# AdrianoEttari/DiffusionRemoteSensing

Measured on AMD Instinct MI355X. Metric: unet_denoise_steps_per_s, higher is better.
Workload: dtype f16 main + block-scaled fp6 (e2m3) cross terms of tap pairs on the wide 3x3 layers (FL, 11 of 11 launches of the dominant kernel); split bf16 x3 (hi + lo) everywhere else; f32 accumulate

## Files before the change

diffusionremotesensing_amd/csrc/reverse_step.hip:

```cpp
#include "drs_common.h"
#include "step_update.h"

__global__ __launch_bounds__(256) void sampler_step_tab_kernel(float* __restrict__ x, const float* __restrict__ eps,
                                                               const float* __restrict__ noise, int t,
                                                               const float* __restrict__ alpha,
                                                               const float* __restrict__ alpha_hat,
                                                               const float* __restrict__ beta, int64_t numel) {
  const DrsAncestralCoef k = drs_ancestral_coef(alpha, alpha_hat, beta, t);
  for (int64_t i = (int64_t)blockIdx.x * blockDim.x + threadIdx.x; i < numel; i += (int64_t)gridDim.x * blockDim.x) {
    float v = drs_ancestral_update(k, x[i], eps[i]);
    if (noise) v = drs_ancestral_noise(k, v, noise[i]);
    x[i] = v;
  }
}

extern "C" int drs_sampler_step(float* x, const float* eps_pred, const float* noise, int t, const float* alpha,
                                const float* alpha_hat, const float* beta, int noise_steps, int64_t numel,
                                drs_stream_t stream) {
  DRS_REQUIRE(x && eps_pred && alpha && alpha_hat && beta, DRS_ERR_ARG, "sampler_step: null pointer");
  if (int st = drs_check_move("sampler_step", false, 0, t, 0, 0.f, noise_steps, noise, DRS_NOISE_OPTIONAL)) return st;
  if (numel <= 0) return DRS_OK;
  DRS_LAUNCH(sampler_step_tab_kernel, dim3(ew_blocks(numel)), dim3(256), 0, (hipStream_t)stream, x, eps_pred,
                     noise, t, alpha, alpha_hat, beta, numel);
  DRS_CHECK_HIP(hipGetLastError());
  return DRS_OK;
}

__global__ void sampler_step_cfg_kernel(float* __restrict__ x, const float* __restrict__ ec,
                                        const float* __restrict__ eu, float w, const float* __restrict__ noise, int t,
                                        const float* __restrict__ alpha, const float* __restrict__ alpha_hat,
                                        const float* __restrict__ beta, int64_t numel) {
  const DrsAncestralCoef k = drs_ancestral_coef(alpha, alpha_hat, beta, t);
  for (int64_t i = (int64_t)blockIdx.x * blockDim.x + threadIdx.x; i < numel; i += (int64_t)gridDim.x * blockDim.x) {
    float v = drs_ancestral_update(k, x[i], drs_cfg_lerp(eu[i], ec[i], w));
    if (noise) v = drs_ancestral_noise(k, v, noise[i]);
    x[i] = v;
  }
}
extern "C" int drs_sampler_step_cfg(float* x, const float* eps_cond, const float* eps_uncond, float cfg_scale,
                                    const float* noise, int t, const float* alpha, const float* alpha_hat,
                                    const float* beta, int noise_steps, int64_t numel, drs_stream_t stream) {
  DRS_REQUIRE(x && eps_cond && eps_uncond && alpha && alpha_hat && beta, DRS_ERR_ARG, "sampler_step_cfg: null pointer");
  if (int st = drs_check_move("sampler_step_cfg", false, 0, t, 0, 0.f, noise_steps, noise, DRS_NOISE_OPTIONAL)) return st;
  if (numel <= 0) return DRS_OK;
  DRS_LAUNCH(sampler_step_cfg_kernel, dim3(ew_blocks(numel)), dim3(256), 0, (hipStream_t)stream, x, eps_cond,
                     eps_uncond, cfg_scale, noise, t, alpha, alpha_hat, beta, numel);
  DRS_CHECK_HIP(hipGetLastError());
  return DRS_OK;
}

namespace {

__global__ __launch_bounds__(256) void ddim_step_kernel(float* __restrict__ x, const float* __restrict__ ec,
                                                        const float* __restrict__ eu, float w,
                                                        const float* __restrict__ noise, int t, int t_prev, float eta,
                                                        const float* __restrict__ alpha_hat, int64_t numel) {
  const DrsDdimCoef k = drs_ddim_coef(alpha_hat, t, t_prev, eta);
  const bool add_noise = noise != nullptr && k.has_sigma;
  for (int64_t i = (int64_t)blockIdx.x * blockDim.x + threadIdx.x; i < numel; i += (int64_t)gridDim.x * blockDim.x) {
    float e = ec[i];
    if (eu) e = drs_cfg_lerp(eu[i], e, w);
    float v = drs_ddim_update(k, x[i], e);
    if (add_noise) v = drs_ddim_noise(k, v, noise[i]);
    x[i] = v;
  }
}

__device__ __forceinline__ float cfg_lerp(float uncond, float cond, float w) {
#pragma clang fp contract(off)
  const float d = cond - uncond;
  return fabsf(w) < 0.5f ? fmaf(w, d, uncond) : fmaf(-(1.f - w), d, cond);
}

template <bool DDIM>
struct MoveCoef;
template <>
struct MoveCoef<false> {
  DrsAncestralCoef k;
  __device__ MoveCoef(const float* alpha, const float* alpha_hat, const float* beta, int t, int, float)
      : k(drs_ancestral_coef(alpha, alpha_hat, beta, t)) {}
  __device__ bool draws() const { return true; }
  __device__ float step(float x, float eps) const {
#pragma clang fp contract(off)
    return k.c_inv * fmaf(-k.c_eps, eps, x);
  }
  __device__ float add(float v, float z) const { return fmaf(k.c_sig, z, v); }
};
template <>
struct MoveCoef<true> {
  DrsDdimCoef k;
  __device__ MoveCoef(const float*, const float* alpha_hat, const float*, int t, int t_prev, float eta)
      : k(drs_ddim_coef(alpha_hat, t, t_prev, eta)) {}
  __device__ bool draws() const { return k.has_sigma; }
  __device__ float step(float x, float eps) const {
#pragma clang fp contract(off)
    const float p = k.a * x, q = k.b * eps;
    return p + q;
  }
  __device__ float add(float v, float z) const { return fmaf(k.s, z, v); }
};

struct InpaintArgs {
  float* x;
  const float* ec;
  const float* eu;
  float w;
  const float* noise;
  const float* known;
  const unsigned char* mask;
  int planes, C, Cm;
  int64_t hw;
  int t, t_prev;
  float eta;
  const float *alpha, *alpha_hat, *beta;
};

template <int V, bool DDIM>
__global__ __launch_bounds__(256) void inpaint_step_kernel(const InpaintArgs a) {
  const MoveCoef<DDIM> coef(a.alpha, a.alpha_hat, a.beta, a.t, a.t_prev, a.eta);
  const DrsKnownCoef kc(a.alpha_hat, a.t_prev);
  const bool add_noise = a.noise != nullptr && coef.draws();
  const bool to_zero = a.t_prev == 0;
  const int64_t groups = a.hw / V;
  for (int plane = blockIdx.y; plane < a.planes; plane += gridDim.y) {
    const int64_t base = (int64_t)plane * a.hw;
    const unsigned char* mp = a.mask + (a.Cm == 1 ? (int64_t)(plane / a.C) * a.hw : base);
    for (int64_t g = (int64_t)blockIdx.x * blockDim.x + threadIdx.x; g < groups; g += (int64_t)gridDim.x * blockDim.x) {
      const int64_t at = base + g * V;
      float xs[V], es[V], ks[V], zs[V];
      unsigned m;
      if constexpr (V == 4) {
        const float4 x4 = *reinterpret_cast<const float4*>(a.x + at);
        const float4 e4 = *reinterpret_cast<const float4*>(a.ec + at);
        const float4 k4 = *reinterpret_cast<const float4*>(a.known + at);
        xs[0] = x4.x; xs[1] = x4.y; xs[2] = x4.z; xs[3] = x4.w;
        es[0] = e4.x; es[1] = e4.y; es[2] = e4.z; es[3] = e4.w;
        ks[0] = k4.x; ks[1] = k4.y; ks[2] = k4.z; ks[3] = k4.w;
        if (a.eu) {
          const float4 u4 = *reinterpret_cast<const float4*>(a.eu + at);
          es[0] = cfg_lerp(u4.x, es[0], a.w); es[1] = cfg_lerp(u4.y, es[1], a.w);
          es[2] = cfg_lerp(u4.z, es[2], a.w); es[3] = cfg_lerp(u4.w, es[3], a.w);
        }
        if (a.noise) {
          const float4 z4 = *reinterpret_cast<const float4*>(a.noise + at);
          zs[0] = z4.x; zs[1] = z4.y; zs[2] = z4.z; zs[3] = z4.w;
        }
        m = *reinterpret_cast<const unsigned*>(mp + g * 4);
      } else {
        xs[0] = a.x[at];
        es[0] = a.ec[at];
        ks[0] = a.known[at];
        if (a.eu) es[0] = cfg_lerp(a.eu[at], es[0], a.w);
        if (a.noise) zs[0] = a.noise[at];
        m = mp[g];
      }
#pragma unroll
      for (int p = 0; p < V; ++p) {
        float v = coef.step(xs[p], es[p]);
        if (add_noise) v = coef.add(v, zs[p]);
        if ((m >> (8 * p)) & 0xffu) v = to_zero ? ks[p] : kc.at(ks[p], zs[p]);
        xs[p] = v;
      }
      if constexpr (V == 4) *reinterpret_cast<float4*>(a.x + at) = make_float4(xs[0], xs[1], xs[2], xs[3]);
      else a.x[at] = xs[0];
    }
  }
}

__device__ __forceinline__ float jump_to(float A, float x, float B, float z) {
#pragma clang fp contract(off)
  const float p = A * x, q = B * z;
  return p + q;
}

__global__ __launch_bounds__(256) void renoise_kernel(float* __restrict__ x, const float* __restrict__ z, int s, int t,
                                                      const float* __restrict__ alpha_hat, int64_t numel, bool vec) {
  const double r = (double)alpha_hat[t] / (double)alpha_hat[s];
  const float A = (float)sqrt(r), B = (float)sqrt(fmax(1.0 - r, 0.0));
  const int64_t tid = (int64_t)blockIdx.x * blockDim.x + threadIdx.x, stride = (int64_t)gridDim.x * blockDim.x;
  const int64_t groups = vec ? numel / 4 : 0;
  for (int64_t g = tid; g < groups; g += stride) {
    float4 v = reinterpret_cast<const float4*>(x)[g];
    const float4 n = reinterpret_cast<const float4*>(z)[g];
    v.x = jump_to(A, v.x, B, n.x);
    v.y = jump_to(A, v.y, B, n.y);
    v.z = jump_to(A, v.z, B, n.z);
    v.w = jump_to(A, v.w, B, n.w);
    reinterpret_cast<float4*>(x)[g] = v;
  }
  for (int64_t i = groups * 4 + tid; i < numel; i += stride) x[i] = jump_to(A, x[i], B, z[i]);
}

__global__ __launch_bounds__(256) void dpm_step_kernel(float* __restrict__ x, const float* __restrict__ ec,
                                                       const float* __restrict__ eu, float w, float* __restrict__ hist,
                                                       int t_q, int t, int t_p, const float* __restrict__ alpha_hat,
                                                       int64_t numel, bool vec) {
  const DrsDpmCoef k = drs_dpm_coef(alpha_hat, t_q, t, t_p);
  const int64_t tid = (int64_t)blockIdx.x * blockDim.x + threadIdx.x, stride = (int64_t)gridDim.x * blockDim.x;
  const int64_t groups = vec ? numel / 4 : 0;
  for (int64_t g = tid; g < groups; g += stride) {
    const float4 x4 = reinterpret_cast<const float4*>(x)[g];
    const float4 e4 = reinterpret_cast<const float4*>(ec)[g];
    float xs[4] = {x4.x, x4.y, x4.z, x4.w}, es[4] = {e4.x, e4.y, e4.z, e4.w}, hs[4] = {0.f, 0.f, 0.f, 0.f};
    if (eu) {
      const float4 u4 = reinterpret_cast<const float4*>(eu)[g];
      es[0] = drs_cfg_lerp(u4.x, es[0], w); es[1] = drs_cfg_lerp(u4.y, es[1], w);
      es[2] = drs_cfg_lerp(u4.z, es[2], w); es[3] = drs_cfg_lerp(u4.w, es[3], w);
    }
    if (k.second) {
      const float4 h4 = reinterpret_cast<const float4*>(hist)[g];
      hs[0] = h4.x; hs[1] = h4.y; hs[2] = h4.z; hs[3] = h4.w;
    }
#pragma unroll
    for (int p = 0; p < 4; ++p) {
      const float x0 = drs_dpm_x0(k, xs[p], es[p]);
      xs[p] = drs_dpm_update(k, xs[p], es[p], hs[p]);
      hs[p] = x0;
    }
    reinterpret_cast<float4*>(hist)[g] = make_float4(hs[0], hs[1], hs[2], hs[3]);
    reinterpret_cast<float4*>(x)[g] = make_float4(xs[0], xs[1], xs[2], xs[3]);
  }
  for (int64_t i = groups * 4 + tid; i < numel; i += stride) {
    float e = ec[i];
    if (eu) e = drs_cfg_lerp(eu[i], e, w);
    const float xv = x[i], h = k.second ? hist[i] : 0.f;
    hist[i] = drs_dpm_x0(k, xv, e);
    x[i] = drs_dpm_update(k, xv, e, h);
  }
}

template <bool DDIM>
int launch_inpaint(const InpaintArgs& a, hipStream_t s) {
  const bool wide = a.hw % 4 == 0 && aligned16(a.x) && aligned16(a.ec) && aligned16(a.known) && ((uintptr_t)a.mask & 3u) == 0 &&
                    (!a.eu || aligned16(a.eu)) && (!a.noise || aligned16(a.noise));
  const int gx = ew_blocks(wide ? a.hw / 4 : a.hw);
  int gy = 8192 / gx;
  if (gy > a.planes) gy = a.planes;
  if (gy < 1) gy = 1;
  if (wide) DRS_LAUNCH((inpaint_step_kernel<4, DDIM>), dim3(gx, gy), dim3(256), 0, s, a);
// ... 67 lines not shown
```

diffusionremotesensing_amd/csrc/small_kernels.hip:

```cpp
#include "drs_common.h"
#include <algorithm>

typedef unsigned u32x4 __attribute__((ext_vector_type(4)));

__global__ void pack_conv_kernel(const float* __restrict__ w, const float* __restrict__ b,
                                 const float* __restrict__ gamma, const float* __restrict__ beta,
                                 const float* __restrict__ rmean, const float* __restrict__ rvar, float eps,
                                 float* __restrict__ dst_w, float* __restrict__ dst_b, int Cout, int Cin, int taps,
                                 int transposed, int mfma_layout) {
  const int64_t total = (int64_t)Cout * Cin * taps;
  for (int64_t i = (int64_t)blockIdx.x * blockDim.x + threadIdx.x; i < total;
       i += (int64_t)gridDim.x * blockDim.x) {
    int tap, ci, co;
    if (mfma_layout) {
      ci = (int)(i % Cin);
      co = (int)((i / Cin) % Cout);
      tap = (int)(i / ((int64_t)Cin * Cout));
    } else {
      co = (int)(i % Cout);
      ci = (int)((i / Cout) % Cin);
      tap = (int)(i / ((int64_t)Cin * Cout));
    }
    const int64_t src = transposed ? (((int64_t)ci * Cout + co) * taps + tap) : (((int64_t)co * Cin + ci) * taps + tap);
    float v = w[src];
// ... 46 lines not shown
    const int c = (int)((i / hw) % C);
    const int n = (int)(i / (hw * C));
    dst[i] = src[((int64_t)n * hw + r) * src_cs + src_co + c];
  }
}
__global__ void sp_to_nchw_kernel(const char* __restrict__ src, float* __restrict__ dst, int N, int C, int H, int W,
                                  int src_cs, int src_co) {
  const int64_t total = (int64_t)N * C * H * W;
  const int64_t hw = (int64_t)H * W;
  const int gw = src_cs >= 32 ? 32 : src_cs;
  for (int64_t i = (int64_t)blockIdx.x * blockDim.x + threadIdx.x; i < total; i += (int64_t)gridDim.x * blockDim.x) {
    const int64_t r = i % hw;
    const int c = (int)((i / hw) % C) + src_co;
    const int n = (int)(i / (hw * C));
    const char* g = src + (((int64_t)n * hw + r) * src_cs + (c / gw) * gw) * 4;
    const __bf16 h = *reinterpret_cast<const __bf16*>(g + (c % gw) * 2);
    const __bf16 l = *reinterpret_cast<const __bf16*>(g + gw * 2 + (c % gw) * 2);
    dst[i] = (float)h + (float)l;
  }
}
__global__ void sp_add_rowvec_kernel(const char* __restrict__ src, char* __restrict__ dst, const float* __restrict__ vec,
                                     int vec_stride, int64_t slots, int64_t slots_per_image, int C) {
  typedef __bf16 bf16x8_t __attribute__((ext_vector_type(8)));
  const int spp = C / 8;
  for (int64_t i = (int64_t)blockIdx.x * blockDim.x + threadIdx.x; i < slots; i += (int64_t)gridDim.x * blockDim.x) {
    const int64_t pix = i / spp;
    const int sl = (int)(i % spp), grp = sl >> 2, kg = sl & 3;
    const int n = (int)(i / slots_per_image);
    const int64_t off = (pix * C + grp * 32) * 4 + kg * 16;
    const bf16x8_t h = *reinterpret_cast<const bf16x8_t*>(src + off), l = *reinterpret_cast<const bf16x8_t*>(src + off + 64);
    const float* v = vec + (int64_t)n * vec_stride + grp * 32 + kg * 8;
    float x[8];
#pragma unroll
    for (int j = 0; j < 8; ++j) x[j] = (float)h[j] + (float)l[j] + v[j];
    u32x4 oh, ol;
#pragma unroll
    for (int q = 0; q < 4; ++q) { const uint2 s_ = drs_split2(x[2 * q], x[2 * q + 1]); oh[q] = s_.x; ol[q] = s_.y; }
    *reinterpret_cast<u32x4*>(dst + off) = oh;
    *reinterpret_cast<u32x4*>(dst + off + 64) = ol;
  }
}
int drs_launch_nchw_to_nhwc(const float* src, float* dst, int N, int C, int H, int W, int dst_cs, int dst_co,
                            hipStream_t s) {
  DRS_LAUNCH(nchw_to_nhwc_kernel, dim3(ew_blocks((int64_t)N * C * H * W)), dim3(256), 0, s, src, dst, N, C, H,
                     W, dst_cs, dst_co);
  DRS_CHECK_HIP(hipGetLastError());
  return DRS_OK;
}
int drs_launch_sp_to_nchw(const float* src, float* dst, int N, int C, int H, int W, int src_cs, int src_co,
                          hipStream_t s) {
  DRS_LAUNCH(sp_to_nchw_kernel, dim3(ew_blocks((int64_t)N * C * H * W)), dim3(256), 0, s,
                     reinterpret_cast<const char*>(src), dst, N, C, H, W, src_cs, src_co);
  DRS_CHECK_HIP(hipGetLastError());
  return DRS_OK;
}
int drs_launch_sp_add_rowvec(const float* src, float* dst, const float* vec, int vec_stride, int N, long long pix_per_image,
                             int C, hipStream_t s) {
  DRS_REQUIRE(C % 32 == 0, DRS_ERR_SHAPE, "sp_add_rowvec: C=%d", C);
  const int64_t per_image = (int64_t)pix_per_image * (C / 8), slots = per_image * N;
  if (slots == 0) return DRS_OK;
  DRS_LAUNCH(sp_add_rowvec_kernel, dim3(ew_blocks(slots)), dim3(256), 0, s, reinterpret_cast<const char*>(src),
                     reinterpret_cast<char*>(dst), vec, vec_stride, slots, per_image, C);
  DRS_CHECK_HIP(hipGetLastError());
  return DRS_OK;
}
int drs_launch_nhwc_to_nchw(const float* src, float* dst, int N, int C, int H, int W, int src_cs, int src_co,
                            hipStream_t s) {
  DRS_LAUNCH(nhwc_to_nchw_kernel, dim3(ew_blocks((int64_t)N * C * H * W)), dim3(256), 0, s, src, dst, N, C, H,
                     W, src_cs, src_co);
  DRS_CHECK_HIP(hipGetLastError());
  return DRS_OK;
}

__global__ __launch_bounds__(256) void conv3x3_planar_kernel(const float* __restrict__ in, const float* __restrict__ w,
                                                             const float* __restrict__ b,
                                                             const float* __restrict__ res, float* __restrict__ out,
                                                             int N, int Cin, int Cout, int H, int W, int relu) {
  constexpr int kW = kMaxBands * kMaxBands * 9;
  __shared__ float sw[kW + kMaxBands];
  for (int i = threadIdx.x; i < Cout * Cin * 9; i += blockDim.x) sw[i] = w[i];
  if (threadIdx.x < Cout) sw[kW + threadIdx.x] = b ? b[threadIdx.x] : 0.f;
  __syncthreads();
  const int64_t hw = (int64_t)H * W;
  const int64_t total = (int64_t)N * hw;
  for (int64_t p = (int64_t)blockIdx.x * blockDim.x + threadIdx.x; p < total; p += (int64_t)gridDim.x * blockDim.x) {
    const int x = (int)(p % W);
    const int y = (int)((p / W) % H);
    const int n = (int)(p / hw);
#pragma unroll 1
    for (int c0 = 0; c0 < Cout; c0 += 4) {
      const int nc = min(4, Cout - c0);
      const float* swc = sw + c0 * Cin * 9;
      float acc[4];
#pragma unroll
      for (int co = 0; co < 4; ++co) acc[co] = co < nc ? sw[kW + c0 + co] : 0.f;
      for (int ci = 0; ci < Cin; ++ci) {
        const float* ip = in + ((int64_t)n * Cin + ci) * hw;
#pragma unroll
        for (int ky = 0; ky < 3; ++ky) {
          const int iy = y + ky - 1;
          if (iy < 0 || iy >= H) continue;
#pragma unroll
          for (int kx = 0; kx < 3; ++kx) {
            const int ix = x + kx - 1;
            if (ix < 0 || ix >= W) continue;
            const float a = ip[(int64_t)iy * W + ix];
#pragma unroll
            for (int co = 0; co < 4; ++co)
              if (co < nc) acc[co] = fmaf(a, swc[(co * Cin + ci) * 9 + ky * 3 + kx], acc[co]);
          }
        }
      }
#pragma unroll
      for (int co = 0; co < 4; ++co) {
        if (co >= nc) break;
        float v = acc[co];
        if (relu) v = drs_maxf(v, 0.f);
        const int64_t o = ((int64_t)n * Cout + c0 + co) * hw + (int64_t)y * W + x;
        if (res) v += res[o];
        out[o] = v;
      }
    }
  }
}
int drs_launch_conv3x3_planar(const float* in, const float* w, const float* b, const float* res, float* out, int N,
                              int Cin, int Cout, int H, int W, int relu, hipStream_t s) {
  DRS_REQUIRE(Cin >= 1 && Cin <= kMaxBands && Cout >= 1 && Cout <= kMaxBands, DRS_ERR_SHAPE,
              "planar conv: Cin=%d Cout=%d (max %d)", Cin, Cout, kMaxBands);
  DRS_LAUNCH(conv3x3_planar_kernel, dim3(ew_blocks((int64_t)N * H * W)), dim3(256), 0, s, in, w, b, res, out,
                     N, Cin, Cout, H, W, relu);
  DRS_CHECK_HIP(hipGetLastError());
  return DRS_OK;
}

constexpr int kStemRows = 4;
constexpr int kStemBpc = 2;
__device__ __attribute__((aligned(16))) float stem_zero_line[4];
template <int COUT>
__global__ __launch_bounds__(256, kStemBpc) void stem_kernel(const float* __restrict__ in, const float* __restrict__ w,
                                                             const float* __restrict__ b, const float* __restrict__ res,
                                                             int res_batch, float* __restrict__ out, int N, int Cin, int H,
                                                             int W, int out_sp) {
  static_assert(COUT == 16, "a pixel is 64 bytes in both output formats");
  constexpr int R = kStemRows;
  constexpr int kB = COUT * kMaxBands * 9;
  __shared__ __attribute__((aligned(16))) float sw[kB + COUT];
  __shared__ __attribute__((aligned(16))) char sT[4][64 * 64];
  for (int i = threadIdx.x; i < COUT * Cin * 9; i += blockDim.x) {
    const int co = i / (Cin * 9), r = i % (Cin * 9), ci = r / 9, tap = r % 9;
    sw[(tap * Cin + ci) * COUT + co] = w[i];
  }
  if (threadIdx.x < COUT) sw[kB + threadIdx.x] = b[threadIdx.x];
  __syncthreads();
  const int lane = threadIdx.x & 63, wave = threadIdx.x >> 6;
  char* tb = sT[wave];
  const int sw_px = (lane >> 2) & 3;
  const int lin_q = (lane & 3) ^ ((lane >> 4) & 3);
  const int lin_off = (lane >> 2) * 64 + lin_q * 16;
  const int64_t hw = (int64_t)H * W;
  const int xbs = (W + 63) / 64, ygs = (H + R - 1) / R;
  const int units = N * ygs * xbs;
  for (int u = blockIdx.x * 4 + wave; u < units; u += gridDim.x * 4) {
    const int xb = u % xbs, yg = (u / xbs) % ygs, n = u / (xbs * ygs);
    const int x0 = xb * 64, x = x0 + lane, y0 = yg * R;
    const int npx = min(64, W - x0);
    float acc[R][COUT];
#pragma unroll
    for (int o = 0; o < R; ++o)
#pragma unroll
      for (int co = 0; co < COUT; ++co) acc[o][co] = sw[kB + co];
    u32x4 rnext[4] = {};
    auto load_res = [&](int o) __attribute__((always_inline)) {
      const int y = min(y0 + o, H - 1);
      const char* rp = reinterpret_cast<const char*>(res + (res_batch == 1 ? ((int64_t)y * W + x0) : ((int64_t)n * H + y) * W + x0) * COUT);
#pragma unroll
      for (int j = 0; j < 4; ++j)
        rnext[j] = *reinterpret_cast<const u32x4*>((j * 16 + (lane >> 2) < npx) ? rp + j * 1024 + lin_off
                                                                                 : reinterpret_cast<const char*>(stem_zero_line));
    };
    if (res) load_res(0);
#pragma unroll 1
    for (int ci = 0; ci < Cin; ++ci) {
      const float* ip = in + ((int64_t)n * Cin + ci) * hw;
      float a[R + 2][3];
#pragma unroll
      for (int r = 0; r < R + 2; ++r) {
        const int iy = y0 - 1 + r;
        const bool yok = iy >= 0 && iy < H;
        const float* rowp = ip + (int64_t)iy * W;
#pragma unroll
        for (int kx = 0; kx < 3; ++kx) {
          const int ix = x - 1 + kx;
          a[r][kx] = *((yok && ix >= 0 && ix < W) ? rowp + ix : stem_zero_line);
        }
      }
#pragma unroll
      for (int ky = 0; ky < 3; ++ky)
#pragma unroll
        for (int kx = 0; kx < 3; ++kx) {
          const float* wr = &sw[((ky * 3 + kx) * Cin + ci) * COUT];
          float wv[COUT];
#pragma unroll
          for (int co = 0; co < COUT; co += 4) {
            const float4 q = *reinterpret_cast<const float4*>(wr + co);
            wv[co] = q.x; wv[co + 1] = q.y; wv[co + 2] = q.z; wv[co + 3] = q.w;
          }
#pragma unroll
          for (int o = 0; o < R; ++o)
#pragma unroll
            for (int co = 0; co < COUT; ++co) acc[o][co] = fmaf(a[o + ky][kx], wv[co], acc[o][co]);
        }
    }
#pragma unroll
    for (int o = 0; o < R; ++o) {
      const int y = y0 + o;
      if (y >= H) break;
      const int64_t p0 = ((int64_t)n * H + y) * W + x0;
      if (res) {
        const u32x4 rv[4] = {rnext[0], rnext[1], rnext[2], rnext[3]};
        if (o + 1 < R) load_res(o + 1);
#pragma unroll
        for (int j = 0; j < 4; ++j) *reinterpret_cast<u32x4*>(tb + j * 1024 + lane * 16) = rv[j];
        asm volatile("s_waitcnt lgkmcnt(0)" ::: "memory");
#pragma unroll
        for (int q = 0; q < 4; ++q) {
          const float4 r4 = *reinterpret_cast<const float4*>(tb + lane * 64 + ((q ^ sw_px) << 4));
          acc[o][q * 4] += r4.x; acc[o][q * 4 + 1] += r4.y; acc[o][q * 4 + 2] += r4.z; acc[o][q * 4 + 3] += r4.w;
        }
        asm volatile("s_waitcnt lgkmcnt(0)" ::: "memory");
      }
      if (out_sp) {
#pragma unroll
        for (int co = 0; co < COUT; co += 8) {
          u32x4 h, l;
#pragma unroll
          for (int q = 0; q < 4; ++q) { const uint2 s_ = drs_split2(acc[o][co + 2 * q], acc[o][co + 2 * q + 1]); h[q] = s_.x; l[q] = s_.y; }
          *reinterpret_cast<u32x4*>(tb + lane * 64 + (((co >> 3) ^ sw_px) << 4)) = h;
          *reinterpret_cast<u32x4*>(tb + lane * 64 + (((2 + (co >> 3)) ^ sw_px) << 4)) = l;
        }
      } else {
#pragma unroll
        for (int co = 0; co < COUT; co += 4)
          *reinterpret_cast<float4*>(tb + lane * 64 + (((co >> 2) ^ sw_px) << 4)) = make_float4(acc[o][co], acc[o][co + 1], acc[o][co + 2], acc[o][co + 3]);
      }
      asm volatile("s_waitcnt lgkmcnt(0)" ::: "memory");
      char* op = reinterpret_cast<char*>(out + p0 * COUT);
#pragma unroll
      for (int j = 0; j < 4; ++j) {
        const u32x4 v = *reinterpret_cast<const u32x4*>(tb + j * 1024 + lane * 16);
        if (j * 16 + (lane >> 2) < npx) *reinterpret_cast<u32x4*>(op + j * 1024 + lin_off) = v;
      }
      asm volatile("s_waitcnt lgkmcnt(0)" ::: "memory");
    }
  }
}
int drs_launch_stem(const float* in_nchw, const float* w, const float* b, const float* res_nhwc, int res_batch,
                    float* out_nhwc, int N, int Cin, int Cout, int H, int W, hipStream_t s, int out_sp) {
  DRS_REQUIRE(Cout == 16 && Cin >= 1 && Cin <= kMaxBands, DRS_ERR_SHAPE, "stem: Cin=%d Cout=%d unsupported (Cin max %d)", Cin,
              Cout, kMaxBands);
  const int64_t units = (int64_t)N * ((H + kStemRows - 1) / kStemRows) * ((W + 63) / 64);
  if (units == 0) return DRS_OK;
  DRS_REQUIRE(units < (1LL << 31), DRS_ERR_SHAPE, "stem: %lld row segments", (long long)units);
  const int64_t blocks = std::min<int64_t>((units + 3) / 4, 16384);
  DRS_LAUNCH(stem_kernel<16>, dim3((unsigned)blocks), dim3(256), 0, s, in_nchw, w, b, res_nhwc,
                     res_batch, out_nhwc, N, Cin, H, W, out_sp);
  DRS_CHECK_HIP(hipGetLastError());
  return DRS_OK;
}

__device__ __forceinline__ void cubic_coeffs(float t, float c[4]) {
  const float A = -0.75f;
  const float x0 = t + 1.f, x1 = t, x2 = 1.f - t, x3 = 2.f - t;
  c[0] = ((A * x0 - 5.f * A) * x0 + 8.f * A) * x0 - 4.f * A;
  c[1] = ((A + 2.f) * x1 - (A + 3.f)) * x1 * x1 + 1.f;
  c[2] = ((A + 2.f) * x2 - (A + 3.f)) * x2 * x2 + 1.f;
  c[3] = ((A * x3 - 5.f * A) * x3 + 8.f * A) * x3 - 4.f * A;
}
__global__ __launch_bounds__(256) void bicubic_kernel(const float* __restrict__ x, float* __restrict__ y, int NC, int H,
                                                      int W, int scale) {
  const int OH = H * scale, OW = W * scale;
  const int64_t total = (int64_t)NC * OH * OW;
  const float rs = 1.f / (float)scale;
  for (int64_t i = (int64_t)blockIdx.x * blockDim.x + threadIdx.x; i < total; i += (int64_t)gridDim.x * blockDim.x) {
    const int ox = (int)(i % OW);
    const int oy = (int)((i / OW) % OH);
    const int64_t nc = i / ((int64_t)OW * OH);
    const float sy = rs * ((float)oy + 0.5f) - 0.5f;
    const float sx = rs * ((float)ox + 0.5f) - 0.5f;
    const float fy = floorf(sy), fx = floorf(sx);
    const int iy = (int)fy, ix = (int)fx;
    float cy[4], cx[4];
    cubic_coeffs(sy - fy, cy);
    cubic_coeffs(sx - fx, cx);
    const float* ip = x + nc * (int64_t)H * W;
    float acc = 0.f;
#pragma unroll
    for (int a = 0; a < 4; ++a) {
      const int yy = min(max(iy - 1 + a, 0), H - 1);
      float row = 0.f;
#pragma unroll
      for (int bq = 0; bq < 4; ++bq) {
        const int xx = min(max(ix - 1 + bq, 0), W - 1);
        row = fmaf(ip[(int64_t)yy * W + xx], cx[bq], row);
      }
      acc = fmaf(row, cy[a], acc);
    }
    y[i] = acc;
  }
}
int drs_launch_bicubic(const float* x, float* y, int N, int C, int H, int W, int scale, hipStream_t s) {
  DRS_REQUIRE(scale >= 1, DRS_ERR_SHAPE, "bicubic: scale=%d", scale);
  DRS_LAUNCH(bicubic_kernel, dim3(ew_blocks((int64_t)N * C * H * W * scale * scale)), dim3(256), 0, s, x, y,
                     N * C, H, W, scale);
  DRS_CHECK_HIP(hipGetLastError());
  return DRS_OK;
}

__global__ __launch_bounds__(256) void time_mlp_kernel(const int64_t* __restrict__ t, const float* __restrict__ inv_freq,
                                                       const float* __restrict__ W1, const float* __restrict__ b1,
                                                       const float* __restrict__ W2, const float* __restrict__ b2,
                                                       float* __restrict__ out, int out_stride, int dim_in,
                                                       int dim_out) {
  extern __shared__ __attribute__((aligned(16))) float smem[];
  float* e = smem;
  float* h = smem + dim_in;
  const int b = blockIdx.x;
  const float tf = (float)t[b];
  const int half = dim_in / 2;
  for (int j = threadIdx.x; j < half; j += blockDim.x) {
    const float arg = tf * inv_freq[j];
    e[j] = sinf(arg);
    e[half + j] = cosf(arg);
  }
  __syncthreads();
  for (int c = threadIdx.x; c < dim_out; c += blockDim.x) {
    const float* wr = W1 + (int64_t)c * dim_in;
    float acc = 0.f;
    for (int k = 0; k < dim_in; ++k) acc = fmaf(wr[k], e[k], acc);
    acc += b1[c];
    h[c] = acc / (1.f + expf(-acc));
  }
  __syncthreads();
  for (int c = threadIdx.x; c < dim_out; c += blockDim.x) {
    const float* wr = W2 + (int64_t)c * dim_out;
    float acc = 0.f;
    for (int k = 0; k < dim_out; ++k) acc = fmaf(wr[k], h[k], acc);
    acc += b2[c];
    out[(int64_t)b * out_stride + c] = drs_maxf(acc, 0.f);
  }
}
int drs_launch_time_mlp(const int64_t* t, const float* inv_freq, const float* W1, const float* b1, const float* W2,
                        const float* b2, float* out, int out_stride, int B, int dim_in, int dim_out, hipStream_t s) {
  DRS_REQUIRE(dim_in % 2 == 0 && dim_in > 0 && dim_out > 0, DRS_ERR_SHAPE, "time_mlp: dims %d %d", dim_in, dim_out);
  if (B == 0) return DRS_OK;
  const size_t shmem = (size_t)(dim_in + dim_out) * sizeof(float);
  DRS_LAUNCH(time_mlp_kernel, dim3(B), dim3(256), shmem, s, t, inv_freq, W1, b1, W2, b2, out, out_stride,
                     dim_in, dim_out);
  DRS_CHECK_HIP(hipGetLastError());
  return DRS_OK;
}

__global__ __launch_bounds__(256) void time_mlp_multi_kernel(const int64_t* __restrict__ t,
                                                             const float* __restrict__ inv_freq,
                                                             const char* __restrict__ packed,
                                                             const long long* __restrict__ table,
                                                             float* __restrict__ out, int out_stride, int dim_in,
                                                             const float* __restrict__ label_emb,
                                                             const long long* __restrict__ labels, int label_batch,
                                                             int num_classes) {
  extern __shared__ __attribute__((aligned(16))) float smem[];
  float* e = smem;
  float* h = smem + dim_in;
  const int b = blockIdx.x;
// ... 200 lines not shown
```

diffusionremotesensing_amd/csrc/upfuse_proj_sp.hip:

```cpp
#include <stdio.h>
#include <stdlib.h>

#include "conv_epilogue.h"
#include "mfma_policy.h"

namespace {

constexpr int RBC = 8;
struct RowOpU { PolicyBF16X3::Frag c, e; };

__device__ __forceinline__ bf16x8 dpp_shift_u(const bf16x8& edge, const bf16x8& own, bool left) {
  const u32x4 e = __builtin_bit_cast(u32x4, edge), r = __builtin_bit_cast(u32x4, own);
  u32x4 o;
#pragma unroll
  for (int j = 0; j < 4; ++j)
    o[j] = left ? (unsigned)__builtin_amdgcn_update_dpp((int)e[j], (int)r[j], 0x111, 0xf, 0xf, false)
                : (unsigned)__builtin_amdgcn_update_dpp((int)e[j], (int)r[j], 0x101, 0xf, 0xf, false);
  return __builtin_bit_cast(bf16x8, o);
}
__host__ __device__ constexpr int up_tap_p(int j) { return j >= 3 ? 1 : 0; }
__host__ __device__ constexpr int up_tap_t(int j) { return j >= 3 ? j - 2 : j; }
__host__ __device__ constexpr bool up_pair(int p, int t, int kv, int kw) { return p + kv - kw == 2 * (t - 1); }

template <int NCK>
__global__ __launch_bounds__(256, 3) void upfuse_proj_sp_kernel(UpFuseDesc d) {
  extern __shared__ __attribute__((aligned(16))) char smem[];
  using P = PolicyBF16X3;
  using Frag = typename P::Frag;
  constexpr int NR = RBC + 2, PF = 2;
  const int tid = threadIdx.x, lane = tid & 63, wave = __builtin_amdgcn_readfirstlane(tid >> 6);
  const int lr = lane & 15, kg = lane >> 4;
  constexpr int IMG = NCK * 5 * 4 * 16 * 16;
  char* sW = smem;
  float* sB = reinterpret_cast<float*>(smem + 2 * IMG);
  {
    const char* w = reinterpret_cast<const char*>(d.w);
    for (int o = tid * 16; o < 2 * IMG; o += 256 * 16) *reinterpret_cast<u32x4*>(sW + o) = *reinterpret_cast<const u32x4*>(w + o);
    if (tid < 4) sB[tid] = d.bias[min(tid, 3) * 8];
  }
  __syncthreads();
  const int OH = 2 * d.LH, OW = 2 * d.LW;
  const int gx = (d.LW + 15) >> 4, gy = (d.LH + RBC - 1) / RBC;
  const int total = d.N * gy * gx;
  const int xcd = blockIdx.x & 7, member = blockIdx.x >> 3, members = gridDim.x >> 3;
  const int t_lo = (int)((long long)total * xcd / 8), t_hi = (int)((long long)total * (xcd + 1) / 8);
  const int stride = members * 4, first = member * 4 + wave;
  const int pixb = d.in_cs * 4;
  const char* zero = reinterpret_cast<const char*>(d.zero_line) + kg * 16;
  const char* wlane = sW + ((size_t)kg * 16 + lr) * 16;
  const size_t plane = (size_t)OH * OW;
  const float bk = sB[kg];
  const int ko = min(kg, d.fuse_dim - 1);
  for (int q0 = t_lo + first; q0 < t_hi; q0 += stride) {
    int q = q0;
    const int x0 = (q % gx) * 16; q /= gx;
    const int m0 = (q % gy) * RBC;
    const int n = q / gy;
    const int cx = x0 + lr;
    const bool own_ok = cx < d.LW && kg < d.fuse_dim;
    RowOpU R[PF + 1][NCK];
    auto load_row = [&](int slot, int wr) __attribute__((always_inline)) {
      const int iy = m0 - 1 + wr;
      const bool ok = iy >= 0 && iy < d.LH && cx < d.LW;
      const char* base = reinterpret_cast<const char*>(d.in) +
                         ((((long long)n * d.LH + iy) * d.LW + cx) * d.in_cs + d.in_co) * 4 + kg * 16;
#pragma unroll
      for (int c = 0; c < NCK; ++c) {
        const char* p = ok ? base + c * 128 : zero;
        R[slot][c].c = Frag{*reinterpret_cast<const bf16x8*>(p), *reinterpret_cast<const bf16x8*>(ok ? p + 64 : zero)};
      }
      if (lr == 0 || lr == 15) {
        const int ex = lr == 0 ? x0 - 1 : x0 + 16;
        const bool eok = iy >= 0 && iy < d.LH && ex >= 0 && ex < d.LW;
        const char* be = reinterpret_cast<const char*>(d.in) +
                         ((((long long)n * d.LH + iy) * d.LW + ex) * d.in_cs + d.in_co) * 4 + kg * 16;
#pragma unroll
        for (int c = 0; c < NCK; ++c) {
          const char* pe = eok ? be + c * 128 : zero;
          R[slot][c].e = Frag{*reinterpret_cast<const bf16x8*>(pe), *reinterpret_cast<const bf16x8*>(eok ? pe + 64 : zero)};
        }
      }
      (void)pixb;
    };
    float* obase = d.fuse_out + ((size_t)n * d.fuse_dim + ko) * plane + 2 * min(cx, d.LW - 1);
    f32x4 S[3][2];
#pragma unroll
    for (int i = 0; i < PF; ++i) load_row(i, i);
#pragma unroll
    for (int wr = 0; wr < NR; ++wr) {
      if (wr + PF < NR) load_row((wr + PF) % (PF + 1), wr + PF);
      __builtin_amdgcn_sched_barrier(0);
      f32x4 s0 = {0.f, 0.f, 0.f, 0.f}, s1 = {0.f, 0.f, 0.f, 0.f};
#pragma unroll
      for (int c = 0; c < NCK; ++c) {
        const RowOpU& r = R[wr % (PF + 1)][c];
#pragma unroll
        for (int tx = 0; tx < 3; ++tx) {
          const Frag a = tx == 1 ? r.c : Frag{dpp_shift_u(r.e.hi, r.c.hi, tx == 0), dpp_shift_u(r.e.lo, r.c.lo, tx == 0)};
          const int g0 = tx == 0 ? 0 : (tx == 1 ? 1 : 3);
          s0 = P::mma(P::load(wlane, (size_t)IMG, (size_t)((c * 5 + g0) * 4 * 16) * 16), a, s0);
          if (tx >= 1) s1 = P::mma(P::load(wlane, (size_t)IMG, (size_t)((c * 5 + g0 + 1) * 4 * 16) * 16), a, s1);
        }
      }
      S[wr % 3][0] = s0;
      S[wr % 3][1] = s1;
      __builtin_amdgcn_sched_barrier(0);
      if (wr >= 2) {
        const int m = m0 + wr - 2;
        const f32x4(&A)[2] = S[(wr - 2) % 3];
        const f32x4(&B)[2] = S[(wr - 1) % 3];
        const f32x4(&C)[2] = S[wr % 3];
        float v[2][2][3];
#pragma unroll
        for (int px = 0; px < 2; ++px)
#pragma unroll
          for (int o = 0; o < 3; ++o) {
            auto pick = [&](const f32x4& t, int row) __attribute__((always_inline)) { return __shfl(t[row & 3], lr + 16 * (row >> 2), 64); };
            v[0][px][o] = pick(A[px], 0 + o) + pick(B[px], 3 + o) + pick(C[px], 6 + o);
            v[1][px][o] = pick(B[px], 9 + o) + pick(C[px], 12 + o);
          }
        if (m < d.LH) {
#pragma unroll
          for (int py = 0; py < 2; ++py) {
            const int oy = 2 * m + py;
            float w0 = kg == 0 ? v[py][0][0] : (kg == 1 ? v[py][0][1] : v[py][0][2]);
            float w1 = kg == 0 ? v[py][1][0] : (kg == 1 ? v[py][1][1] : v[py][1][2]);
            float2* op = reinterpret_cast<float2*>(obase + (size_t)oy * OW);
            float2 prev = make_float2(0.f, 0.f);
            if (own_ok && d.fuse_acc) prev = *op;
            w0 += bk + prev.x;
            w1 += bk + prev.y;
            if (d.eh && own_ok) {
              const int ch = ko * 8;
              if (oy == 0 || oy == OH - 1) {
                const float* e = d.eh + (((size_t)n * 2 + (oy ? 1 : 0)) * OW + 2 * cx) * d.Ch + ch;
                w0 += e[0];
                w1 += e[d.Ch];
              } else {
                if (cx == 0) w0 += d.ev[(((size_t)n * 2 + 0) * OH + oy) * d.Ch + ch];
                if (2 * cx + 1 == OW - 1) w1 += d.ev[(((size_t)n * 2 + 1) * OH + oy) * d.Ch + ch];
              }
            }
            if (own_ok) *op = make_float2(w0, w1);
          }
        }
      }
    }
  }
}

__global__ __launch_bounds__(128) void upfuse_proj_pack_kernel(const float* __restrict__ vp, const float* __restrict__ t_w, int Cc,
                                                               int Ch, int fuse_dim, char* __restrict__ dst) {
  const int nck = Cc >> 5;
  const int nslots = nck * 5 * 4 * 16;
  const size_t img = (size_t)nslots * 16;
  const int cinv = Cc + Ch;
  for (int s = blockIdx.x * 128 + threadIdx.x; s < nslots; s += gridDim.x * 128) {
    const int row = s & 15, q = (s >> 4) & 3, g = (s >> 6) % 5, ck = s / 320;
    const int j = row / 3, o = row - 3 * j;
    float x[8] = {0.f, 0.f, 0.f, 0.f, 0.f, 0.f, 0.f, 0.f};
    if (row < 15 && o < fuse_dim) {
      const int tx = g == 0 ? 0 : (g <= 2 ? 1 : 2), px = (g == 2 || g == 4) ? 1 : 0, py = up_tap_p(j), ty = up_tap_t(j);
      const int ci0 = ck * 32 + q * 8;
      for (int kvy = 0; kvy < 3; ++kvy)
        for (int kwy = 0; kwy < 3; ++kwy) {
          if (!up_pair(py, ty, kvy, kwy)) continue;
          for (int kvx = 0; kvx < 3; ++kvx)
            for (int kwx = 0; kwx < 3; ++kwx) {
              if (!up_pair(px, tx, kvx, kwx)) continue;
              const float* vq = vp + (size_t)(8 * o) * cinv * 9 + kvy * 3 + kvx;
              const float* wq = t_w + (size_t)ci0 * Cc * 9 + kwy * 3 + kwx;
              for (int c = 0; c < Cc; ++c) {
                const float vv = vq[(size_t)c * 9];
#pragma unroll
                for (int e = 0; e < 8; ++e) x[e] += vv * wq[((size_t)e * Cc + c) * 9];
              }
            }
        }
    }
    PolicyBF16X3::cvt_store(dst, img, (size_t)s * 16, x);
  }
}

}

size_t drs_upfuse_proj_weight_bytes(int Cc) { return (size_t)2 * (Cc / 32) * 5 * 4 * 16 * 16; }

bool drs_upfuse_proj_supported(int Cc, int Ch, int fuse_dim) {
  return Ch == 32 && (Cc == 32 || Cc == 64) && fuse_dim >= 1 && fuse_dim <= 3;
}

int drs_launch_upfuse_proj_pack(const float* vp, const float* t_w, int Cc, int Ch, int fuse_dim, void* dst, hipStream_t s) {
  DRS_REQUIRE(vp && t_w && dst && drs_upfuse_proj_supported(Cc, Ch, fuse_dim), DRS_ERR_SHAPE, "upfuse_proj_pack: Cc=%d Ch=%d fuse_dim=%d", Cc, Ch, fuse_dim);
  const int nslots = (Cc / 32) * 5 * 4 * 16;
  DRS_LAUNCH(upfuse_proj_pack_kernel, dim3((nslots + 127) / 128), dim3(128), 0, s, vp, t_w, Cc, Ch, fuse_dim, (char*)dst);
  DRS_CHECK_HIP(hipGetLastError());
  return DRS_OK;
}

int drs_launch_upfuse_proj(const UpFuseDesc& d, hipStream_t s) {
  DRS_REQUIRE(d.in && d.w && d.bias && d.zero_line && d.fuse_out && d.proj && !d.res && !d.out && !d.out2, DRS_ERR_ARG, "upfuse_proj: bad descriptor");
  DRS_REQUIRE(drs_upfuse_proj_supported(d.Cc, d.Ch, d.fuse_dim) && (d.in_cs & 31) == 0 && (d.in_co & 31) == 0, DRS_ERR_SHAPE, "upfuse_proj: channels");
  DRS_REQUIRE((d.eh == nullptr) == (d.ev == nullptr), DRS_ERR_ARG, "upfuse_proj: edge vectors");
  if ((size_t)d.N * d.LH * d.LW == 0) return DRS_OK;
  int num_cu = 0;
  const void* kern = d.Cc == 64 ? reinterpret_cast<const void*>(upfuse_proj_sp_kernel<2>) : reinterpret_cast<const void*>(upfuse_proj_sp_kernel<1>);
  {
    const int rc = drs_kernel_prepare(kern, 0, &num_cu);
    if (rc) return rc;
  }
  const size_t lds = drs_upfuse_proj_weight_bytes(d.Cc) + 64;
  const long long strips = (long long)d.N * ((d.LH + RBC - 1) / RBC) * ((d.LW + 15) >> 4);
  long long blocks = (long long)num_cu * 3;
  if (blocks * 4 > strips) blocks = (strips + 3) / 4;
  blocks = (blocks + 7) / 8 * 8;
  if (d.Cc == 64) DRS_LAUNCH(upfuse_proj_sp_kernel<2>, dim3((unsigned)blocks), dim3(256), lds, s, d);
  else DRS_LAUNCH(upfuse_proj_sp_kernel<1>, dim3((unsigned)blocks), dim3(256), lds, s, d);
  DRS_CHECK_HIP(hipGetLastError());
  return DRS_OK;
}
```

Before: 820.6.

## Vectorize sampler step, prefetch stem conv taps, and prefetch fused-output accumulators

```diff
diff --git a/diffusionremotesensing_amd/csrc/reverse_step.hip b/diffusionremotesensing_amd/csrc/reverse_step.hip
--- a/diffusionremotesensing_amd/csrc/reverse_step.hip
+++ b/diffusionremotesensing_amd/csrc/reverse_step.hip
@@ -1,15 +1,39 @@
 #include "drs_common.h"
 #include "step_update.h"
+
+__device__ __forceinline__ float ancestral_step(const DrsAncestralCoef& k, float x, float eps) {
+#pragma clang fp contract(off)
+  return k.c_inv * fmaf(-k.c_eps, eps, x);
+}
+__device__ __forceinline__ float ancestral_add(const DrsAncestralCoef& k, float v, float z) { return fmaf(k.c_sig, z, v); }
 
 __global__ __launch_bounds__(256) void sampler_step_tab_kernel(float* __restrict__ x, const float* __restrict__ eps,
                                                                const float* __restrict__ noise, int t,
                                                                const float* __restrict__ alpha,
                                                                const float* __restrict__ alpha_hat,
-                                                               const float* __restrict__ beta, int64_t numel) {
+                                                               const float* __restrict__ beta, int64_t numel, bool vec) {
   const DrsAncestralCoef k = drs_ancestral_coef(alpha, alpha_hat, beta, t);
-  for (int64_t i = (int64_t)blockIdx.x * blockDim.x + threadIdx.x; i < numel; i += (int64_t)gridDim.x * blockDim.x) {
-    float v = drs_ancestral_update(k, x[i], eps[i]);
-    if (noise) v = drs_ancestral_noise(k, v, noise[i]);
+  const int64_t tid = (int64_t)blockIdx.x * blockDim.x + threadIdx.x, stride = (int64_t)gridDim.x * blockDim.x;
+  const int64_t groups = vec ? numel / 4 : 0;
+  for (int64_t g = tid; g < groups; g += stride) {
+    float4 v = reinterpret_cast<const float4*>(x)[g];
+    const float4 e = reinterpret_cast<const float4*>(eps)[g];
+    v.x = ancestral_step(k, v.x, e.x);
+    v.y = ancestral_step(k, v.y, e.y);
+    v.z = ancestral_step(k, v.z, e.z);
+    v.w = ancestral_step(k, v.w, e.w);
+    if (noise) {
+      const float4 z = reinterpret_cast<const float4*>(noise)[g];
+      v.x = ancestral_add(k, v.x, z.x);
+      v.y = ancestral_add(k, v.y, z.y);
+      v.z = ancestral_add(k, v.z, z.z);
+      v.w = ancestral_add(k, v.w, z.w);
+    }
+    reinterpret_cast<float4*>(x)[g] = v;
+  }
+  for (int64_t i = groups * 4 + tid; i < numel; i += stride) {
+    float v = ancestral_step(k, x[i], eps[i]);
+    if (noise) v = ancestral_add(k, v, noise[i]);
     x[i] = v;
   }
 }
@@ -20,8 +44,9 @@
   DRS_REQUIRE(x && eps_pred && alpha && alpha_hat && beta, DRS_ERR_ARG, "sampler_step: null pointer");
   if (int st = drs_check_move("sampler_step", false, 0, t, 0, 0.f, noise_steps, noise, DRS_NOISE_OPTIONAL)) return st;
   if (numel <= 0) return DRS_OK;
-  DRS_LAUNCH(sampler_step_tab_kernel, dim3(ew_blocks(numel)), dim3(256), 0, (hipStream_t)stream, x, eps_pred,
-                     noise, t, alpha, alpha_hat, beta, numel);
+  const bool vec = aligned16(x) && aligned16(eps_pred) && (!noise || aligned16(noise));
+  DRS_LAUNCH(sampler_step_tab_kernel, dim3(ew_blocks(vec ? (numel + 3) / 4 : numel)), dim3(256), 0, (hipStream_t)stream, x, eps_pred,
+                     noise, t, alpha, alpha_hat, beta, numel, vec);
   DRS_CHECK_HIP(hipGetLastError());
   return DRS_OK;
 }
@@ -80,11 +105,8 @@
   __device__ MoveCoef(const float* alpha, const float* alpha_hat, const float* beta, int t, int, float)
       : k(drs_ancestral_coef(alpha, alpha_hat, beta, t)) {}
   __device__ bool draws() const { return true; }
-  __device__ float step(float x, float eps) const {
-#pragma clang fp contract(off)
-    return k.c_inv * fmaf(-k.c_eps, eps, x);
-  }
-  __device__ float add(float v, float z) const { return fmaf(k.c_sig, z, v); }
+  __device__ float step(float x, float eps) const { return ancestral_step(k, x, eps); }
+  __device__ float add(float v, float z) const { return ancestral_add(k, v, z); }
 };
 template <>
 struct MoveCoef<true> {
diff --git a/diffusionremotesensing_amd/csrc/small_kernels.hip b/diffusionremotesensing_amd/csrc/small_kernels.hip
--- a/diffusionremotesensing_amd/csrc/small_kernels.hip
+++ b/diffusionremotesensing_amd/csrc/small_kernels.hip
@@ -222,7 +222,7 @@
   }
   if (threadIdx.x < COUT) sw[kB + threadIdx.x] = b[threadIdx.x];
   __syncthreads();
-  const int lane = threadIdx.x & 63, wave = threadIdx.x >> 6;
+  const int lane = threadIdx.x & 63, wave = __builtin_amdgcn_readfirstlane(threadIdx.x >> 6);
   char* tb = sT[wave];
   const int sw_px = (lane >> 2) & 3;
   const int lin_q = (lane & 3) ^ ((lane >> 4) & 3);
@@ -239,47 +239,61 @@
     for (int o = 0; o < R; ++o)
 #pragma unroll
       for (int co = 0; co < COUT; ++co) acc[o][co] = sw[kB + co];
-    u32x4 rnext[4] = {};
+    constexpr int RD = 1;
+    u32x4 rres[RD][4] = {};
     auto load_res = [&](int o) __attribute__((always_inline)) {
       const int y = min(y0 + o, H - 1);
       const char* rp = reinterpret_cast<const char*>(res + (res_batch == 1 ? ((int64_t)y * W + x0) : ((int64_t)n * H + y) * W + x0) * COUT);
 #pragma unroll
       for (int j = 0; j < 4; ++j)
-        rnext[j] = *reinterpret_cast<const u32x4*>((j * 16 + (lane >> 2) < npx) ? rp + j * 1024 + lin_off
+        rres[o % RD][j] = *reinterpret_cast<const u32x4*>((j * 16 + (lane >> 2) < npx) ? rp + j * 1024 + lin_off
                                                                                  : reinterpret_cast<const char*>(stem_zero_line));
     };
-    if (res) load_res(0);
+    const unsigned xc[3] = {4u * (unsigned)min(max(x - 1, 0), W - 1), 4u * (unsigned)min(x, W - 1), 4u * (unsigned)min(x + 1, W - 1)};
+    const bool xok[3] = {x >= 1 && x - 1 < W, x < W, x + 1 < W};
+    float a[R + 2][3], an[R + 2][3];
+    auto load_taps = [&](int ci) __attribute__((always_inline)) {
+      typedef const __attribute__((address_space(1))) char* gptr;
+      gptr ip = (gptr)(in + ((int64_t)n * Cin + ci) * hw);
+      asm volatile("" : "+s"(ip));
+#pragma unroll
+      for (int r = 0; r < R + 2; ++r) {
+        gptr rowp = ip + (int64_t)min(max(y0 - 1 + r, 0), H - 1) * W * 4;
+#pragma unroll
+        for (int kx = 0; kx < 3; ++kx) an[r][kx] = *(const __attribute__((address_space(1))) float*)(rowp + xc[kx]);
+      }
+    };
+    load_taps(0);
+    if (res) {
+#pragma unroll
+      for (int o = 0; o < RD; ++o) load_res(o);
+    }
 #pragma unroll 1
     for (int ci = 0; ci < Cin; ++ci) {
-      const float* ip = in + ((int64_t)n * Cin + ci) * hw;
-      float a[R + 2][3];
 #pragma unroll
       for (int r = 0; r < R + 2; ++r) {
-        const int iy = y0 - 1 + r;
-        const bool yok = iy >= 0 && iy < H;
-        const float* rowp = ip + (int64_t)iy * W;
-#pragma unroll
-        for (int kx = 0; kx < 3; ++kx) {
-          const int ix = x - 1 + kx;
-          a[r][kx] = *((yok && ix >= 0 && ix < W) ? rowp + ix : stem_zero_line);
+        const bool yok = y0 - 1 + r >= 0 && y0 - 1 + r < H;
+#pragma unroll
+        for (int kx = 0; kx < 3; ++kx) a[r][kx] = (yok && xok[kx]) ? an[r][kx] : 0.f;
+      }
+      if (ci + 1 < Cin) load_taps(ci + 1);
+      __builtin_amdgcn_sched_barrier(0);
+#pragma unroll
+      for (int tap = 0; tap < 9; ++tap) {
+        const int ky = tap / 3, kx = tap % 3;
+        const float* wr = &sw[(tap * Cin + ci) * COUT];
+        float wv[COUT];
+#pragma unroll
+        for (int co = 0; co < COUT; co += 4) {
+          const float4 q = *reinterpret_cast<const float4*>(wr + co);
+          wv[co] = q.x; wv[co + 1] = q.y; wv[co + 2] = q.z; wv[co + 3] = q.w;
         }
-      }
-#pragma unroll
-      for (int ky = 0; ky < 3; ++ky)
-#pragma unroll
-        for (int kx = 0; kx < 3; ++kx) {
-          const float* wr = &sw[((ky * 3 + kx) * Cin + ci) * COUT];
-          float wv[COUT];
-#pragma unroll
-          for (int co = 0; co < COUT; co += 4) {
-            const float4 q = *reinterpret_cast<const float4*>(wr + co);
-            wv[co] = q.x; wv[co + 1] = q.y; wv[co + 2] = q.z; wv[co + 3] = q.w;
-          }
-#pragma unroll
-          for (int o = 0; o < R; ++o)
-#pragma unroll
-            for (int co = 0; co < COUT; ++co) acc[o][co] = fmaf(a[o + ky][kx], wv[co], acc[o][co]);
-        }
+#pragma unroll
+        for (int o = 0; o < R; ++o)
+#pragma unroll
+          for (int co = 0; co < COUT; ++co) acc[o][co] = fmaf(a[o + ky][kx], wv[co], acc[o][co]);
+        __builtin_amdgcn_sched_barrier(0);
+      }
     }
 #pragma unroll
     for (int o = 0; o < R; ++o) {
@@ -287,8 +301,8 @@
       if (y >= H) break;
       const int64_t p0 = ((int64_t)n * H + y) * W + x0;
       if (res) {
-        const u32x4 rv[4] = {rnext[0], rnext[1], rnext[2], rnext[3]};
-        if (o + 1 < R) load_res(o + 1);
+        const u32x4 rv[4] = {rres[o % RD][0], rres[o % RD][1], rres[o % RD][2], rres[o % RD][3]};
+        if (o + RD < R) load_res(o + RD);
 #pragma unroll
         for (int j = 0; j < 4; ++j) *reinterpret_cast<u32x4*>(tb + j * 1024 + lane * 16) = rv[j];
         asm volatile("s_waitcnt lgkmcnt(0)" ::: "memory");
diff --git a/diffusionremotesensing_amd/csrc/upfuse_proj_sp.hip b/diffusionremotesensing_amd/csrc/upfuse_proj_sp.hip
--- a/diffusionremotesensing_amd/csrc/upfuse_proj_sp.hip
+++ b/diffusionremotesensing_amd/csrc/upfuse_proj_sp.hip
@@ -27,7 +27,7 @@
   extern __shared__ __attribute__((aligned(16))) char smem[];
   using P = PolicyBF16X3;
   using Frag = typename P::Frag;
-  constexpr int NR = RBC + 2, PF = 2;
+  constexpr int NR = RBC + 2, PF = 2, PD = 1;
   const int tid = threadIdx.x, lane = tid & 63, wave = __builtin_amdgcn_readfirstlane(tid >> 6);
   const int lr = lane & 15, kg = lane >> 4;
   constexpr int IMG = NCK * 5 * 4 * 16 * 16;
@@ -83,11 +83,23 @@
       (void)pixb;
     };
     float* obase = d.fuse_out + ((size_t)n * d.fuse_dim + ko) * plane + 2 * min(cx, d.LW - 1);
+    float2 PV[PD + 1][2];
+    auto load_prev = [&](int wr) __attribute__((always_inline)) {
+      const int m = m0 + wr - 2;
+#pragma unroll
+      for (int py = 0; py < 2; ++py) {
+        PV[wr % (PD + 1)][py] = make_float2(0.f, 0.f);
+        if (own_ok && d.fuse_acc && m < d.LH) PV[wr % (PD + 1)][py] = *reinterpret_cast<const float2*>(obase + (size_t)(2 * m + py) * OW);
+      }
+    };
     f32x4 S[3][2];
 #pragma unroll
     for (int i = 0; i < PF; ++i) load_row(i, i);
 #pragma unroll
+    for (int i = 2; i < PD; ++i) load_prev(i);
+#pragma unroll
     for (int wr = 0; wr < NR; ++wr) {
+      if (wr + PD >= 2 && wr + PD < NR) load_prev(wr + PD);
       if (wr + PF < NR) load_row((wr + PF) % (PF + 1), wr + PF);
       __builtin_amdgcn_sched_barrier(0);
       f32x4 s0 = {0.f, 0.f, 0.f, 0.f}, s1 = {0.f, 0.f, 0.f, 0.f};
@@ -126,8 +138,7 @@
             float w0 = kg == 0 ? v[py][0][0] : (kg == 1 ? v[py][0][1] : v[py][0][2]);
             float w1 = kg == 0 ? v[py][1][0] : (kg == 1 ? v[py][1][1] : v[py][1][2]);
             float2* op = reinterpret_cast<float2*>(obase + (size_t)oy * OW);
-            float2 prev = make_float2(0.f, 0.f);
-            if (own_ok && d.fuse_acc) prev = *op;
+            const float2 prev = PV[wr % (PD + 1)][py];
             w0 += bk + prev.x;
             w1 += bk + prev.y;
             if (d.eh && own_ok) {
```

Result: no change. 825.0, median of 5 (+0.5%).
